# asbschmidt/CUDASW4

Measured on NVIDIA B200. Metric: GCUPS, higher is better.
Workload: dtype s16x2 (DPX) with exact s32 re-scoring

## Files before the change

cudasw4_b200/csrc/kernels_s16.cuh:

```cuda
#pragma once
#include <cstdint>
#include <utility>
#include <cuda_runtime.h>

namespace sw4 {

#ifndef SW4_S16_THREADS
#define SW4_S16_THREADS 512
#endif
constexpr int kS16Threads = SW4_S16_THREADS;
constexpr int kS16Warps = kS16Threads / 32;
constexpr int kRingSlots = 64;
constexpr int kRingStride = 96;
constexpr int kFused = 441;
constexpr int kBatchSteps = 8;
constexpr int kBatchRows = 2 * kBatchSteps;
constexpr int kRingBytes = kFused * kRingStride * 4;
constexpr short kNegS16 = -16000;

struct S16Item {
    int subject0, subject1;
    int firstBlock;
    int numSegments;
};

struct S16Params {
    const uint16_t* cols;
    const S16Item* items;
    int numItems;
    int firstSubject, numSubjects;
    int* ticket;
    int logG;
    const uint32_t* profile;
    int profStride;
    int qlen;
    int period;
    uint32_t gop2, gex2;
    int ovfThreshold;
    int statThreshold;
    int32_t* scores;
    int32_t* ovfList;
    int* ovfCount;
    int* statCount;
    unsigned long long* elapsedNs;
    int activeGroups;
    int ctaOffset;
    const int32_t* lengths;
    uint4* border;
    int borderStride;
    int* borderSlots;
    int numBorderSlots;
    int blockScale;
};

template <int N, class Fn, int... Is>
__device__ __forceinline__ void static_for_impl(Fn&& fn, std::integer_sequence<int, Is...>) {
    (fn(std::integral_constant<int, Is>{}), ...);
}
template <int N, class Fn>
__device__ __forceinline__ void static_for(Fn&& fn) {
    static_for_impl<N>(fn, std::make_integer_sequence<int, N>{});
}

template <int IMM>
__device__ __forceinline__ uint32_t lds_u32_imm(uint32_t addr) {
    uint32_t v;
    asm volatile("ld.shared.u32 %0, [%1+%2];" : "=r"(v) : "r"(addr), "n"(IMM));
    return v;
}
template <int IMM>
__device__ __forceinline__ uint2 lds_u64_imm(uint32_t addr) {
    uint2 v;
    asm volatile("ld.shared.v2.u32 {%0, %1}, [%2+%3];" : "=r"(v.x), "=r"(v.y) : "r"(addr), "n"(IMM));
    return v;
}
__device__ __forceinline__ void cp_async16(uint32_t dst, const void* src) {
    asm volatile("cp.async.cg.shared.global [%0], [%1], 16;" ::"r"(dst), "l"(src));
}
__device__ __forceinline__ void cp_async8(uint32_t dst, const void* src) {
    asm volatile("cp.async.ca.shared.global [%0], [%1], 8;" ::"r"(dst), "l"(src));
}
__device__ __forceinline__ void cp_async4(uint32_t dst, const void* src) {
    asm volatile("cp.async.ca.shared.global [%0], [%1], 4;" ::"r"(dst), "l"(src));
}
__device__ __forceinline__ void cp_async_commit() { asm volatile("cp.async.commit_group;"); }
__device__ __forceinline__ void cp_async_wait_all() { asm volatile("cp.async.wait_group 0;" ::: "memory"); }

constexpr int kStatMaxLength = 8000;
constexpr int kGroupStateInts = 8;

template <int R>
__host__ __device__ constexpr int s16_prefetch_depth() {
#ifdef SW4_S16_PREFETCH
    return SW4_S16_PREFETCH;
#else
    return R == 20 ? 6 : (R == 24 || R == 28 || R == 30) ? 14 : R == 32 ? 7 : 10;
#endif
}

constexpr int kFillPlanBytes = kS16Threads * 8;
__device__ __forceinline__ void ring_fill_plan(uint32_t planBase, uint32_t ringBase, int profStride) {
    const int f0 = threadIdx.x >> 2, c = threadIdx.x & 3;
    const uint32_t dst0 = ringBase + (f0 * kRingStride + 32 + 4 * c) * 4;
    const uint32_t srcOff0 = ((uint32_t)f0 * (uint32_t)profStride + 4u * c) * 4u;
    asm volatile("st.shared.v2.u32 [%0], {%1, %2};" ::"r"(planBase + threadIdx.x * 8), "r"(dst0), "r"(srcOff0) : "memory");
}
__device__ __forceinline__ void ring_fill_fast(uint32_t planBase, const uint32_t* __restrict__ profile, int profStride, int x0, int p0) {
    constexpr int kRowsPerRound = kS16Threads / 4;
    constexpr int kRounds = (kFused + kRowsPerRound - 1) / kRowsPerRound;
    uint32_t dst, srcOff;
    asm volatile("ld.shared.v2.u32 {%0, %1}, [%2];" : "=r"(dst), "=r"(srcOff) : "r"(planBase + threadIdx.x * 8));
    const int slot0 = x0 & (kRingSlots - 1);
    const bool mirror = slot0 >= 32;
    const unsigned char* src = reinterpret_cast<const unsigned char*>(profile) + (srcOff + (uint32_t)p0 * 4u);
    const uint32_t rowStep = (uint32_t)kRowsPerRound * (uint32_t)profStride * 4u;
    dst += slot0 * 4;
#pragma unroll
    for (int k = 0; k < kRounds; k++) {
        if (k < kRounds - 1 || threadIdx.x < (kFused - (kRounds - 1) * kRowsPerRound) * 4) {
            cp_async16(dst + k * (kRowsPerRound * kRingStride * 4), src);
            if (mirror) cp_async16(dst + k * (kRowsPerRound * kRingStride * 4) - kRingSlots * 4, src);
        }
        src += rowStep;
    }
    cp_async_commit();
}

constexpr int kBorderStageBytes = 2 * kBatchSteps * 16;
template <int R, bool MULTI = false>
__host__ __device__ constexpr int s16_smem_bytes() {
    return kRingBytes + kS16Warps * 32 * R * 2 + kS16Warps * 4 * kGroupStateInts * 4 + (MULTI ? kS16Warps * 2 * kBorderStageBytes : 0) +
           kS16Threads * 8;
}

__device__ __forceinline__ void ring_fill(uint32_t ringBase, const uint32_t* __restrict__ profile, int profStride, int x0,
                                          int p0) {
    const int slot0 = x0 & (kRingSlots - 1);
    for (int id = threadIdx.x; id < kFused * (kBatchRows / 4); id += kS16Threads) {
        const int f = id >> 2, c = id & 3;
        const int slot = slot0 + 4 * c;
        const uint32_t* src = profile + (size_t)f * profStride + p0 + 4 * c;
        const uint32_t dst = ringBase + (f * kRingStride + 32 + slot) * 4;
        cp_async16(dst, src);
        if (slot >= 32) cp_async16(dst - kRingSlots * 4, src);
    }
    cp_async_commit();
}

__device__ __forceinline__ uint4 lds_u128(uint32_t addr) {
    uint4 v;
    asm volatile("ld.shared.v4.u32 {%0, %1, %2, %3}, [%4];" : "=r"(v.x), "=r"(v.y), "=r"(v.z), "=r"(v.w) : "r"(addr));
    return v;
}
template <int IMM>
__device__ __forceinline__ uint4 lds_u128_imm(uint32_t addr) {
    uint4 v;
    asm volatile("ld.shared.v4.u32 {%0, %1, %2, %3}, [%4+%5];" : "=r"(v.x), "=r"(v.y), "=r"(v.z), "=r"(v.w) : "r"(addr), "n"(IMM));
    return v;
}
__device__ __forceinline__ void sts_u128(uint32_t addr, uint32_t a, uint32_t b, uint32_t c, uint32_t d) {
    asm volatile("st.shared.v4.u32 [%0], {%1, %2, %3, %4};" ::"r"(addr), "r"(a), "r"(b), "r"(c), "r"(d) : "memory");
}

constexpr int kS16GapSets = 4;
__host__ __device__ constexpr uint2 s16_gap_set(int gaps) {
    return gaps == 1 ? uint2{0xfff5fff5u, 0xffffffffu} : gaps == 2 ? uint2{0xfff3fff3u, 0xfffefffeu}
         : gaps == 3 ? uint2{0xfff6fff6u, 0xffffffffu} : uint2{0u, 0u};
}
inline int s16_gap_set_for(uint32_t gop2, uint32_t gex2) {
    for (int g = 1; g < kS16GapSets; g++)
        if (s16_gap_set(g).x == gop2 && s16_gap_set(g).y == gex2) return g;
    return 0;
}

template <int R, bool MULTI = false, int GAPS = 0>
__global__ void __launch_bounds__(kS16Threads, 1) sw_s16_kernel(const S16Params prm) {
    static_assert(R % 2 == 0, "a lane's staging slice (R u16 codes) must be a whole number of 4-byte words");
    extern __shared__ __align__(16) unsigned char smem[];
    unsigned long long tStart;
    asm volatile("mov.u64 %0, %%globaltimer;" : "=l"(tStart));
    const uint32_t ringBase = (uint32_t)__cvta_generic_to_shared(smem);
    const int lane = threadIdx.x & 31, warp = threadIdx.x >> 5;
    const int hl = lane & 15;
    const int logG = prm.logG, G = 1 << logG;
    const int g = lane >> logG, m = lane & (G - 1);
    const int groupsPerWarp = 32 >> logG;
    const int P = prm.period;
    const int periodRows = 2 * P;
    const unsigned groupMask = ((G == 16 ? 0xffffu : 0xffu)) << (g << logG);
    const int leader = g << logG;
    const uint32_t NEG2 = ((uint32_t)(uint16_t)kNegS16 << 16) | (uint16_t)kNegS16;
    const uint32_t SW4_GOP2 = GAPS > 0 ? s16_gap_set(GAPS).x : prm.gop2;
    const uint32_t SW4_GEX2 = GAPS > 0 ? s16_gap_set(GAPS).y : prm.gex2;

    int borderSlot = 0;
    if constexpr (MULTI) {
        __shared__ int sBorderSlot;
        if (threadIdx.x == 0) {
            unsigned smid;
            asm volatile("mov.u32 %0, %%smid;" : "=r"(smid));
            int i = (int)(smid % (unsigned)prm.numBorderSlots);
            while (atomicCAS(prm.borderSlots + i, 0, 1) != 0) {
                if (++i == prm.numBorderSlots) i = 0;
                __nanosleep(200);
            }
            sBorderSlot = i;
        }
        __syncthreads();
        borderSlot = sBorderSlot;
    }

    if (warp * groupsPerWarp >= prm.activeGroups) {
        for (int i = threadIdx.x; i < kFused * kRingStride; i += kS16Threads) reinterpret_cast<uint32_t*>(smem)[i] = NEG2;
        __syncthreads();
        ring_fill(ringBase, prm.profile, prm.profStride, 0, 0);
        int pf = kBatchRows % periodRows;
#pragma unroll 1
        for (int batch = 0;; ++batch) {
            cp_async_wait_all();
            if (!__syncthreads_or(false)) break;
            ring_fill(ringBase, prm.profile, prm.profStride, (batch + 1) * kBatchRows, pf);
            pf += kBatchRows;
            if (pf >= periodRows) pf -= periodRows;
        }
        return;
    }

    const uint32_t stageLane = ringBase + kRingBytes + (warp * 32 + lane) * (R * 2);
    volatile int* gs = reinterpret_cast<volatile int*>(smem + kRingBytes + kS16Warps * 32 * R * 2) +
                       (warp * 4 + g) * kGroupStateInts;

    uint4* borderBase = nullptr;
    uint32_t bstage = 0;
    if constexpr (MULTI) {
        const size_t groupGlobal = (size_t)borderSlot * (kS16Warps * 2) + warp * 2 + g;
        borderBase = prm.border + groupGlobal * (size_t)prm.borderStride + 16;
        bstage = ringBase + kRingBytes + kS16Warps * 32 * R * 2 + kS16Warps * 4 * kGroupStateInts * 4 + (warp * 2 + g) * kBorderStageBytes;
    }
    bool useBorder = false;
    bool nextUseBorder = false;
    int pl = 0;

    uint32_t colAddr[R];
    uint32_t Hp[R];
    uint32_t F[R];
    uint32_t mx = 0, HlastA = 0, ElastA = NEG2, ElastB = NEG2, HinPrevB = 0;
#pragma unroll
    for (int j = 0; j < R; j++) { colAddr[j] = ringBase; Hp[j] = 0; F[j] = NEG2; }
    int p = (hl == 0) ? 0 : P - hl;
    const int pRestart = (m == 0) ? 0 : P - m;
    bool haveWork = false;
    bool alive = (warp * groupsPerWarp + g) < prm.activeGroups;

    auto fetch_lookahead = [&](bool continuing, int curBlock) {
        int blk = -1, isNew = 0, item = -1;
        if (!alive) {
            item = prm.numItems;
        } else if (continuing) {
            blk = curBlock + 1;
        } else {
            if (m == 0) item = atomicAdd(prm.ticket, 1);
            item = __shfl_sync(groupMask, item, leader);
            if (item < prm.numItems) { blk = MULTI ? prm.items[item].firstBlock * prm.blockScale : item; isNew = 1; }
        }
        if (m == 0) { gs[3] = blk >= 0; gs[4] = blk; gs[5] = isNew; gs[6] = item; }
        if constexpr (MULTI) nextUseBorder = blk >= 0 && !isNew;
        if (blk >= 0) {
            const unsigned char* src = (const unsigned char*)(prm.cols + (size_t)blk * (G * R)) + m * (R * 2);
            if constexpr ((R * 2) % 16 == 0) {
#pragma unroll
                for (int i = 0; i < R * 2 / 16; i++) cp_async16(stageLane + i * 16, src + i * 16);
            } else if constexpr ((R * 2) % 8 == 0) {
#pragma unroll
                for (int i = 0; i < R * 2 / 8; i++) cp_async8(stageLane + i * 8, src + i * 8);
            } else {
#pragma unroll
                for (int i = 0; i < R * 2 / 4; i++) cp_async4(stageLane + i * 4, src + i * 4);
            }
        }
        cp_async_commit();
        __syncwarp(groupMask);
    };

    for (int i = threadIdx.x; i < kFused * kRingStride; i += kS16Threads) reinterpret_cast<uint32_t*>(smem)[i] = NEG2;
    __syncthreads();
    constexpr int kSmemBytes = s16_smem_bytes<R, MULTI>();
    const uint32_t fillPlan = ringBase + kSmemBytes - kFillPlanBytes;
    ring_fill_plan(fillPlan, ringBase, prm.profStride);
    ring_fill_fast(fillPlan, prm.profile, prm.profStride, 0, 0);
    fetch_lookahead(false, 0);
    int pfill = kBatchRows % periodRows;
    if constexpr (MULTI) {
        if (m < kBatchSteps) { sts_u128(bstage + m * 16, 0, NEG2, 0, NEG2); sts_u128(bstage + 128 + m * 16, 0, NEG2, 0, NEG2); }
    }
    bool writeBorder = false;

    uint32_t phaseBase = ringBase + (32 - 2 * hl) * 4;
#pragma unroll 1
    for (int batch = 0;; ++batch) {
        cp_async_wait_all();
        if (!__syncthreads_or(alive)) break;
        ring_fill_fast(fillPlan, prm.profile, prm.profStride, (batch + 1) * kBatchRows, pfill);
        pfill += kBatchRows;
        if (pfill >= periodRows) pfill -= periodRows;
        if (batch > 0) {
            const int delta = (batch & 3) ? kBatchRows * 4 : -(kRingSlots - kBatchRows) * 4;
            phaseBase += delta;
#pragma unroll
            for (int j = 0; j < R; j++) colAddr[j] += delta;
        }
        if (p == pRestart && alive) {
            __syncwarp(groupMask);
            int segsLeft = gs[2];
            if (haveWork && segsLeft == 0) {
                uint32_t r = mx;
                for (int o = G >> 1; o > 0; o >>= 1) r = __vmaxs2(r, __shfl_xor_sync(groupMask, r, o));
                if (m == 0) {
                    const int s0 = gs[0], s1 = gs[1];
                    const int lo = (int)(short)(r & 0xffff), hi = (int)(short)(r >> 16);
                    if (s0 >= 0) {
                        if (lo >= prm.statThreshold && (!MULTI || prm.lengths[s0] <= kStatMaxLength)) atomicAdd(prm.statCount, 1);
                        if (lo >= prm.ovfThreshold) prm.ovfList[atomicAdd(prm.ovfCount, 1)] = s0;
                        prm.scores[s0] = lo;
                    }
                    if (s1 >= 0) {
                        if (hi >= prm.statThreshold && (!MULTI || prm.lengths[s1] <= kStatMaxLength)) atomicAdd(prm.statCount, 1);
                        if (hi >= prm.ovfThreshold) prm.ovfList[atomicAdd(prm.ovfCount, 1)] = s1;
                        prm.scores[s1] = hi;
                    }
                }
            }
            const bool laValid = gs[3] != 0;
            const int laBlk = gs[4];
            const bool laNew = gs[5] != 0;
            haveWork = laValid;
            alive = laValid;
            if constexpr (MULTI) writeBorder = false;
            if (laValid) {
                if (laNew) {
                    S16Item it;
                    if constexpr (MULTI) {
                        it = prm.items[gs[6]];
                    } else {
                        const int k = gs[6];
                        it.subject0 = prm.firstSubject + 2 * k;
                        it.subject1 = (2 * k + 1 < prm.numSubjects) ? it.subject0 + 1 : -1;
                        it.firstBlock = k;
                        it.numSegments = 1;
                    }
                    int nseg = it.numSegments;
                    if constexpr (MULTI) {
                        nseg *= prm.blockScale;
                        if (prm.blockScale > 1) {
                            const int len0 = prm.lengths[it.subject0], len1 = it.subject1 >= 0 ? prm.lengths[it.subject1] : 0;
                            nseg = max(1, min(nseg, (max(len0, len1) + G * R - 1) / (G * R)));
                        }
                    }
                    __syncwarp(groupMask);
                    if (m == 0) { gs[0] = it.subject0; gs[1] = it.subject1; gs[2] = nseg - 1; }
                    segsLeft = nseg - 1;
                    mx = 0;
                } else {
                    __syncwarp(groupMask);
                    if (m == 0) gs[2] = segsLeft - 1;
                    segsLeft -= 1;
                }
                if constexpr (MULTI) { useBorder = !laNew; writeBorder = segsLeft > 0; }
                cp_async_wait_all();
                __syncwarp(groupMask);
#pragma unroll
                for (int b = 0; b < R / 2; b++) {
                    const uint32_t w = lds_u32_imm<0>(stageLane + b * 4);
                    colAddr[b * 2 + 0] = phaseBase + (w & 0xffffu) * (kRingStride * 4);
                    colAddr[b * 2 + 1] = phaseBase + (w >> 16) * (kRingStride * 4);
                }
#pragma unroll
                for (int j = 0; j < R; j++) { Hp[j] = 0; F[j] = NEG2; }
                HinPrevB = 0; HlastA = 0; ElastA = NEG2; ElastB = NEG2;
                __syncwarp(groupMask);
                fetch_lookahead(segsLeft > 0, laBlk);
            }
        }
        uint32_t bstageRd = 0;
        uint4* borderWr = nullptr;
        bool wb15 = false;
        if constexpr (MULTI) {
            const int plNext = (pl + kBatchSteps >= P) ? 0 : pl + kBatchSteps;
            const bool ub = (plNext == 0) ? nextUseBorder : useBorder;
            if (m < kBatchSteps) {
                const uint32_t dst = bstage + ((batch + 1) & 1) * (kBatchSteps * 16) + m * 16;
                if (ub && 2 * (plNext + m) < prm.qlen) cp_async16(dst, borderBase + plNext + m);
                else sts_u128(dst, 0, NEG2, 0, NEG2);
            }
            cp_async_commit();
            bstageRd = bstage + (batch & 1) * (kBatchSteps * 16);
            borderWr = borderBase + (pl - (G - 1));
            wb15 = writeBorder && m == G - 1;
        }
        static_for<kBatchSteps>([&](auto stepIndex) {
            constexpr int i = decltype(stepIndex)::value;
            uint32_t HinA = __shfl_up_sync(0xffffffffu, HlastA, 1);
            uint32_t EinA = __shfl_up_sync(0xffffffffu, ElastA, 1);
            uint32_t HinB = __shfl_up_sync(0xffffffffu, Hp[R - 1], 1);
            uint32_t EinB = __shfl_up_sync(0xffffffffu, ElastB, 1);
            if constexpr (MULTI) {
                const uint4 bv = lds_u128_imm<i * 16>(bstageRd);
                if (m == 0) { HinA = bv.x; EinA = bv.y; HinB = bv.z; EinB = bv.w; }
            } else {
                if (m == 0) { HinA = 0; EinA = NEG2; HinB = 0; EinB = NEG2; }
            }
            {
                uint32_t E1 = EinA, E2 = EinB;
                constexpr int kPrefetch = s16_prefetch_depth<R>();
                uint2 sq[kPrefetch + 1];
#pragma unroll
                for (int c = 0; c <= kPrefetch && c < R; c++) sq[c] = lds_u64_imm<i * 8>(colAddr[c]);
                uint32_t da = __vadd2(HinPrevB, sq[0].x);
                uint32_t db = __vadd2(HinA, sq[0].y);
                uint32_t ha = 0;
#pragma unroll
                for (int j = 0; j < R; j++) {
                    const uint2 sn = sq[(j + 1) % (kPrefetch + 1)];
                    if (j + 1 + kPrefetch < R) sq[j % (kPrefetch + 1)] = lds_u64_imm<i * 8>(colAddr[j + 1 + kPrefetch]);
                    uint32_t na = 0, nb = 0;
                    if (j + 1 < R) na = __vadd2(Hp[j], sn.x);
                    ha = __vimax3_s16x2_relu(da, E1, F[j]);
                    const uint32_t ta = __vadd2(ha, SW4_GOP2);
                    E1 = __viaddmax_s16x2(E1, SW4_GEX2, ta);
                    const uint32_t Fa = __viaddmax_s16x2(F[j], SW4_GEX2, ta);
                    if (j + 1 < R) nb = __vadd2(ha, sn.y);
                    const uint32_t hb = __vimax3_s16x2_relu(db, E2, Fa);
                    Hp[j] = hb;
                    const uint32_t tb = __vadd2(hb, SW4_GOP2);
                    E2 = __viaddmax_s16x2(E2, SW4_GEX2, tb);
                    F[j] = __viaddmax_s16x2(Fa, SW4_GEX2, tb);
                    mx = __vimax3_s16x2(mx, da, db);
                    da = na;
                    db = nb;
                }
                HlastA = ha;
                ElastA = E1;
                ElastB = E2;
                HinPrevB = HinB;
            }
            if constexpr (MULTI) {
                if (wb15) borderWr[i] = make_uint4(HlastA, ElastA, Hp[R - 1], ElastB);
            }
        });
        p += kBatchSteps;
        if (p >= P) p -= P;
        if constexpr (MULTI) pl = (pl + kBatchSteps >= P) ? 0 : pl + kBatchSteps;
    }
    if (threadIdx.x == 0) {
        unsigned long long tEnd;
        asm volatile("mov.u64 %0, %%globaltimer;" : "=l"(tEnd));
        atomicMax(prm.elapsedNs, tEnd - tStart);
        atomicMax(prm.elapsedNs + 32, ~tStart);
        atomicMax(prm.elapsedNs + 64, tEnd);
        if constexpr (MULTI) {
            __threadfence();
            atomicExch(prm.borderSlots + borderSlot, 0);
        }
    }
}

}
```

Baseline: 8232.

## Overlap column-index fetch with ring wait and drop per-batch column address updates

Moves the cp.async wait and block barrier after the per-group restart handling, so the lookahead column fetch is committed in the same group and only the previous group is waited on (wait_group 1). Replaces the per-batch increment of all R column addresses with a phase offset computed from batch&3 and added at each shared load. Ring fill copies become predicated cp.async, and the restart check uses a countdown. This aims to cut register updates and barrier stalls per batch, but it changes cp.async grouping semantics and adds an add per load.

```diff
diff --git a/cudasw4_b200/csrc/kernels_s16.cuh b/cudasw4_b200/csrc/kernels_s16.cuh
--- a/cudasw4_b200/csrc/kernels_s16.cuh
+++ b/cudasw4_b200/csrc/kernels_s16.cuh
@@ -77,6 +77,10 @@
 __device__ __forceinline__ void cp_async16(uint32_t dst, const void* src) {
     asm volatile("cp.async.cg.shared.global [%0], [%1], 16;" ::"r"(dst), "l"(src));
 }
+__device__ __forceinline__ void cp_async16_if(bool pred, uint32_t dst, const void* src) {
+    asm volatile("{\n\t.reg .pred p;\n\tsetp.ne.b32 p, %2, 0;\n\t@p cp.async.cg.shared.global [%0], [%1], 16;\n\t}"
+                 ::"r"(dst), "l"(src), "r"((int)pred));
+}
 __device__ __forceinline__ void cp_async8(uint32_t dst, const void* src) {
     asm volatile("cp.async.ca.shared.global [%0], [%1], 8;" ::"r"(dst), "l"(src));
 }
@@ -85,6 +89,7 @@
 }
 __device__ __forceinline__ void cp_async_commit() { asm volatile("cp.async.commit_group;"); }
 __device__ __forceinline__ void cp_async_wait_all() { asm volatile("cp.async.wait_group 0;" ::: "memory"); }
+__device__ __forceinline__ void cp_async_wait_prior() { asm volatile("cp.async.wait_group 1;" ::: "memory"); }
 
 constexpr int kStatMaxLength = 8000;
 constexpr int kGroupStateInts = 8;
@@ -115,12 +120,12 @@
     const unsigned char* src = reinterpret_cast<const unsigned char*>(profile) + (srcOff + (uint32_t)p0 * 4u);
     const uint32_t rowStep = (uint32_t)kRowsPerRound * (uint32_t)profStride * 4u;
     dst += slot0 * 4;
+    const bool last = threadIdx.x < (kFused - (kRounds - 1) * kRowsPerRound) * 4;
 #pragma unroll
     for (int k = 0; k < kRounds; k++) {
-        if (k < kRounds - 1 || threadIdx.x < (kFused - (kRounds - 1) * kRowsPerRound) * 4) {
-            cp_async16(dst + k * (kRowsPerRound * kRingStride * 4), src);
-            if (mirror) cp_async16(dst + k * (kRowsPerRound * kRingStride * 4) - kRingSlots * 4, src);
-        }
+        const bool live = k < kRounds - 1 || last;
+        cp_async16_if(live, dst + k * (kRowsPerRound * kRingStride * 4), src);
+        cp_async16_if(live && mirror, dst + k * (kRowsPerRound * kRingStride * 4) - kRingSlots * 4, src);
         src += rowStep;
     }
     cp_async_commit();
@@ -247,8 +252,9 @@
     uint32_t mx = 0, HlastA = 0, ElastA = NEG2, ElastB = NEG2, HinPrevB = 0;
 #pragma unroll
     for (int j = 0; j < R; j++) { colAddr[j] = ringBase; Hp[j] = 0; F[j] = NEG2; }
-    int p = (hl == 0) ? 0 : P - hl;
+    const int p = (hl == 0) ? 0 : P - hl;
     const int pRestart = (m == 0) ? 0 : P - m;
+    int toRestart = pRestart - p < 0 ? pRestart - p + P : pRestart - p;
     bool haveWork = false;
     bool alive = (warp * groupsPerWarp + g) < prm.activeGroups;
 
@@ -278,7 +284,6 @@
                 for (int i = 0; i < R * 2 / 4; i++) cp_async4(stageLane + i * 4, src + i * 4);
             }
         }
-        cp_async_commit();
         __syncwarp(groupMask);
     };
 
@@ -289,27 +294,17 @@
     ring_fill_plan(fillPlan, ringBase, prm.profStride);
     ring_fill_fast(fillPlan, prm.profile, prm.profStride, 0, 0);
     fetch_lookahead(false, 0);
+    cp_async_commit();
     int pfill = kBatchRows % periodRows;
     if constexpr (MULTI) {
         if (m < kBatchSteps) { sts_u128(bstage + m * 16, 0, NEG2, 0, NEG2); sts_u128(bstage + 128 + m * 16, 0, NEG2, 0, NEG2); }
     }
     bool writeBorder = false;
 
-    uint32_t phaseBase = ringBase + (32 - 2 * hl) * 4;
+    const uint32_t laneBase = ringBase + (32 - 2 * hl) * 4;
 #pragma unroll 1
     for (int batch = 0;; ++batch) {
-        cp_async_wait_all();
-        if (!__syncthreads_or(alive)) break;
-        ring_fill_fast(fillPlan, prm.profile, prm.profStride, (batch + 1) * kBatchRows, pfill);
-        pfill += kBatchRows;
-        if (pfill >= periodRows) pfill -= periodRows;
-        if (batch > 0) {
-            const int delta = (batch & 3) ? kBatchRows * 4 : -(kRingSlots - kBatchRows) * 4;
-            phaseBase += delta;
-#pragma unroll
-            for (int j = 0; j < R; j++) colAddr[j] += delta;
-        }
-        if (p == pRestart && alive) {
+        if (toRestart == 0 && alive) {
             __syncwarp(groupMask);
             int segsLeft = gs[2];
             if (haveWork && segsLeft == 0) {
@@ -371,8 +366,8 @@
 #pragma unroll
                 for (int b = 0; b < R / 2; b++) {
                     const uint32_t w = lds_u32_imm<0>(stageLane + b * 4);
-                    colAddr[b * 2 + 0] = phaseBase + (w & 0xffffu) * (kRingStride * 4);
-                    colAddr[b * 2 + 1] = phaseBase + (w >> 16) * (kRingStride * 4);
+                    colAddr[b * 2 + 0] = laneBase + (w & 0xffffu) * (kRingStride * 4);
+                    colAddr[b * 2 + 1] = laneBase + (w >> 16) * (kRingStride * 4);
                 }
 #pragma unroll
                 for (int j = 0; j < R; j++) { Hp[j] = 0; F[j] = NEG2; }
@@ -381,6 +376,13 @@
                 fetch_lookahead(segsLeft > 0, laBlk);
             }
         }
+        cp_async_commit();
+        cp_async_wait_prior();
+        if (!__any_sync(0xffffffffu, __syncthreads_or(alive))) break;
+        ring_fill_fast(fillPlan, prm.profile, prm.profStride, (batch + 1) * kBatchRows, pfill);
+        pfill += kBatchRows;
+        if (pfill >= periodRows) pfill -= periodRows;
+        const uint32_t phase = (uint32_t)(batch & 3) * (kBatchRows * 4);
         uint32_t bstageRd = 0;
         uint4* borderWr = nullptr;
         bool wb15 = false;
@@ -414,14 +416,14 @@
                 constexpr int kPrefetch = s16_prefetch_depth<R>();
                 uint2 sq[kPrefetch + 1];
 #pragma unroll
-                for (int c = 0; c <= kPrefetch && c < R; c++) sq[c] = lds_u64_imm<i * 8>(colAddr[c]);
+                for (int c = 0; c <= kPrefetch && c < R; c++) sq[c] = lds_u64_imm<i * 8>(colAddr[c] + phase);
                 uint32_t da = __vadd2(HinPrevB, sq[0].x);
                 uint32_t db = __vadd2(HinA, sq[0].y);
                 uint32_t ha = 0;
 #pragma unroll
                 for (int j = 0; j < R; j++) {
                     const uint2 sn = sq[(j + 1) % (kPrefetch + 1)];
-                    if (j + 1 + kPrefetch < R) sq[j % (kPrefetch + 1)] = lds_u64_imm<i * 8>(colAddr[j + 1 + kPrefetch]);
+                    if (j + 1 + kPrefetch < R) sq[j % (kPrefetch + 1)] = lds_u64_imm<i * 8>(colAddr[j + 1 + kPrefetch] + phase);
                     uint32_t na = 0, nb = 0;
                     if (j + 1 < R) na = __vadd2(Hp[j], sn.x);
                     ha = __vimax3_s16x2_relu(da, E1, F[j]);
@@ -447,8 +449,8 @@
                 if (wb15) borderWr[i] = make_uint4(HlastA, ElastA, Hp[R - 1], ElastB);
             }
         });
-        p += kBatchSteps;
-        if (p >= P) p -= P;
+        toRestart -= kBatchSteps;
+        if (toRestart < 0) toRestart += P;
         if constexpr (MULTI) pl = (pl + kBatchSteps >= P) ? 0 : pl + kBatchSteps;
     }
     if (threadIdx.x == 0) {
```

Result: no change. 8262, median of 6 (+0.4%).
